# Tencent-RoboticsX/lifelike-agility-and-play

Measured on NVIDIA H100. Metric: env-steps/sec PMC mocap-tracking, higher is better.
Workload: dtype f32

## Files before the change

### __graft_entry__.py

```python
import os
import subprocess
import sys

ROOT = os.path.dirname(os.path.abspath(__file__))
if ROOT not in sys.path:
    sys.path.insert(0, ROOT)
CSRC = os.path.join(ROOT, "lifelike_agility_and_play_b200", "csrc")
CUDA_LIB = os.path.join(CSRC, "libllq_cuda.so")
NVCC_FLAGS = ["-gencode", "arch=compute_90a,code=sm_90a", "-lineinfo", "-O3", "-std=c++17", "-prec-div=false",
              "-prec-sqrt=false", "-ftz=true", "-Xcompiler", "-fPIC", "-shared"]


def _stale(target, sources):
    if not os.path.exists(target):
        return True
    t = os.path.getmtime(target)
    return any(os.path.getmtime(s) > t for s in sources)


def build(force=False):
    srcs = [os.path.join(CSRC, f) for f in ("llq_cuda.cu", "llq_kernels.cuh", "llq_step16.cuh", "llq_math.cuh")]
    srcs += [os.path.join(ROOT, "include", f) for f in ("llq.h", "llq_model_layout.h")]
    srcs.append(os.path.abspath(__file__))
    if force or _stale(CUDA_LIB, srcs):
        nvcc = os.environ.get("NVCC", "/usr/local/cuda/bin/nvcc")
        subprocess.check_call([nvcc] + NVCC_FLAGS + ["-o", CUDA_LIB, os.path.join(CSRC, "llq_cuda.cu")])
    pol_lib, pol_src = os.path.join(CSRC, "libllq_policy.so"), [os.path.join(CSRC, "llq_policy.cu"), os.path.join(CSRC, "llq_policy_hier.cu")]
    if force or _stale(pol_lib, pol_src + [os.path.join(CSRC, "llq_philox.cuh"), os.path.join(ROOT, "include", "llq_policy.h"),
                                           os.path.join(ROOT, "include", "llq.h"), os.path.abspath(__file__)]):
        nvcc = os.environ.get("NVCC", "/usr/local/cuda/bin/nvcc")
        flags = [f for f in NVCC_FLAGS if not f.startswith("-prec-") and not f.startswith("-ftz")]
        subprocess.check_call([nvcc] + flags + ["-o", pol_lib] + pol_src)
    from oracle import oracle as _oracle
    _oracle.build(force=force)
    import lifelike_agility_and_play_b200

# ... 53 lines not shown
```

### lifelike_agility_and_play_b200/csrc/llq_cuda.cu

```cuda
#include "../../include/llq.h"
#include "../../include/llq_model_layout.h"
#include "llq_kernels.cuh"
#include "llq_step16.cuh"

#include <cmath>
#include <cstdio>
#include <cstdlib>
#include <cstring>
#include <new>
#include <string>
#include <vector>

namespace {

thread_local std::string g_err;
int fail(int code, const std::string& msg) { g_err = msg; return code; }
#define CK(call)                                                                                         \
  do {                                                                                                   \
    cudaError_t e_ = (call);                                                                             \
    if (e_ != cudaSuccess) return fail(LLQ_ECUDA, std::string(#call) + ": " + cudaGetErrorString(e_));   \
  } while (0)

constexpr int kPadFrames = 128;

// ... 70 lines not shown
    h->h_scratch = nullptr; h->d_scratch = nullptr; h->h_scratch_bytes = 0;
    CK(cudaMallocHost(&h->h_scratch, bytes));
    CK(cudaMalloc(&h->d_scratch, bytes));
    h->h_scratch_bytes = h->d_scratch_bytes = bytes;
  }
  return LLQ_OK;
}

llq::MocapDev mocap_dev(llq_handle h) { return llq::MocapDev{h->d_frames, h->d_clip_off, h->n_clips, h->d_ob_table, h->d_ob_off}; }

template <int ENV>
void launch_reset_t(llq_handle h, const llq::EnvArrays& E, const llq::ResetParams& RP, float* obs2, long long ld, cudaStream_t s) {
  constexpr int BLOCK = llq::kResetBlock;
  int threads = 4 * h->cfg.n_envs;
  int grid = (threads + BLOCK - 1) / BLOCK;
  size_t smem = sizeof(double) * (size_t)(h->n_clips > 0 ? h->n_clips : 1);
  llq::pmc_reset_kernel<ENV><<<grid, BLOCK, smem, s>>>(E, mocap_dev(h), h->P, h->d_model, RP, obs2, ld);
}
template <int ENV>
int launch_step16(llq_handle h, const llq::EnvArrays& E, const float* a, float* obs2, long long ld, cudaStream_t s) {
  constexpr int EPB = LLQ16_BLOCK / 16;
  const int grid = (h->cfg.n_envs + EPB - 1) / EPB;
  const size_t smem = sizeof(float) * (EPB * llq::kEnvFloats + (LLQ16_BLOCK / 32) * llq::kATabWarp);
  const unsigned bit = 1u << (16 + ENV);
  if (!(h->smem_attr_set & bit)) {
    CK(cudaFuncSetAttribute(llq::llq_step16_kernel<ENV>, cudaFuncAttributeMaxDynamicSharedMemorySize, (int)smem));
    h->smem_attr_set |= bit;
  }
  llq::llq_step16_kernel<ENV><<<grid, LLQ16_BLOCK, smem, s>>>(E, mocap_dev(h), h->P, h->d_model, h->d_sph, a, obs2, ld, h->d_winner[h->parity],
                                                   (unsigned long long)h->cfg.seed, (long long)h->cfg.global_env_offset, h->record);
  return LLQ_OK;
// ... 630 lines not shown

int llq_sync(llq_handle h) {
  if (!h) return fail(LLQ_EINVAL, "null handle");
  int rc = set_device(h);
  if (rc) return rc;
  CK(cudaStreamSynchronize(h->stream));
  return LLQ_OK;
}

const char* llq_last_error(void) { return g_err.c_str(); }

}

#ifdef LLQ16_TIMING
extern "C" int llq_debug_timing(void* out, int n_warps) {
  return cudaMemcpyFromSymbol(out, llq::g_t16, (size_t)n_warps * 12 * sizeof(unsigned long long)) == cudaSuccess ? 0 : -1;
}
#endif
```

### lifelike_agility_and_play_b200/csrc/llq_kernels.cuh

```cuda
#pragma once
#include "../../include/llq.h"
#include "llq_math.cuh"
#include <cuda_pipeline.h>
#include <stdint.h>

namespace llq {

constexpr int kObsDim = 207, kObsDimEpmc = 916, kObsDimSepmc = 965, kPropDim = 33, kActDim = 12, kStateDim = 37, kAuxDim = 18;
template <int ENV> struct ObsW { static constexpr int value = (ENV == 1 || ENV == 3) ? kObsDimEpmc : (ENV == 2 ? kObsDimSepmc : kObsDim); };
constexpr int kMaxBoxes = 36, kMaxCand = 12;

constexpr int kNewObs = 120;
constexpr int kSQ = 0, kSQd = 12;
constexpr int kSPropBase = 24;
constexpr int kSAct = kPropDim;
constexpr int kSFuture = 45;
constexpr int kSRot = 45;
constexpr int kSPos = 54;
constexpr int kSTarget = 57;
constexpr int kSTargetSpd = 59;
constexpr int kSPosNorm = 60;
constexpr int kSCorrYaw = 61;
constexpr int kSMaskGrid = 62, kSMaskFront = 64, kSMaskLidar = 66;
constexpr int kSFlag = 57;
// ... 442 lines not shown
    snew[kSCorrYaw] = yaw;
    snew[kSMaskGrid] = __uint_as_float((unsigned)m2); snew[kSMaskGrid + 1] = __uint_as_float((unsigned)(m2 >> 32));
    snew[kSMaskFront] = __uint_as_float((unsigned)mf); snew[kSMaskFront + 1] = __uint_as_float((unsigned)(mf >> 32));
    snew[kSMaskLidar] = __uint_as_float((unsigned)m1); snew[kSMaskLidar + 1] = __uint_as_float((unsigned)(m1 >> 32));
  }
}
LLQ_DI unsigned long long staged_mask(const float* sn, int slot) {
  return ((unsigned long long)__float_as_uint(sn[slot + 1]) << 32) | __float_as_uint(sn[slot]);
}

struct ObsCtx {
  KinBase kb;
  float kq[3], kqd[3];
};

LLQ_DI ObsCtx build_obs_new(const MocapDev& mc, const StepParams& P, const ModelConst& M, int lane4, int clip, int frame_id,
                            double frac, double px, double py, double pz, Q4 qb, V3 lin, V3 ang, const float (&q)[3],
                            const float (&qd)[3], float* snew) {
  ObsCtx o;
  const MocapFrame* f0 = mc.frames + mc.clip_off[clip] + frame_id;
  o.kb = mocap_base(f0, f0 + 1, frac, P.frame_dt);
  float inv = (float)(1.0 / P.frame_dt), fr = (float)frac;
#pragma unroll
  for (int i = 0; i < 3; i++) {
    float c = f0->q[3 * lane4 + i], n = f0[1].q[3 * lane4 + i];
    o.kq[i] = fmaf(fr, n - c, c);
    o.kqd[i] = (n - c) * inv;
  }
  qb = qnormalize(qb);
  M3 Rb = qmat(qb);
  stage_joints(snew, lane4, q, qd);
  if (lane4 == 0) stage_prop_base(snew, Rb, tmul(Rb, ang), tmul(Rb, lin));
  {
    const double tf = lane4 == 0 ? 1. / 30. : (lane4 == 1 ? 1. / 15. : (lane4 == 2 ? 1. / 3. : 1.));
    double t = P.frame_dt * frac + tf;
    int fid = (int)floor(t / P.frame_dt);
    double ffrac = t / P.frame_dt - fid;
    const MocapFrame* g0 = f0 + fid;
    KinBase kf = mocap_base(g0, g0 + 1, ffrac, P.frame_dt);
    V3 dp = tmul(Rb, V3{(float)(kf.px - px), (float)(kf.py - py), (float)(kf.pz - pz)});
    V3 rv = q_rotvec(qnormalize(qmul(qconj(qb), qnormalize(kf.q))));
    float angle = norm3(rv);
    float sc = angle / (angle + 1e-8f);
    float* o18 = snew + kSFuture + 18 * lane4;
    o18[0] = dp.x; o18[1] = dp.y; o18[2] = dp.z;
    o18[3] = sc * rv.x; o18[4] = sc * rv.y; o18[5] = sc * rv.z;
    float ff = (float)ffrac;
#pragma unroll
    for (int j = 0; j < 12; j++) { float c = g0->q[j], n = g0[1].q[j]; o18[6 + j] = fmaf(ff, n - c, c); }
  }
  return o;
}

LLQ_DI M3 staged_rot(const float* sn) {
  const float* r = sn + kSRot;
  return M3{r[0], r[1], r[2], r[3], r[4], r[5], r[6], r[7], r[8]};
}
LLQ_DI float2 grid_point(const float* sn, int t) {
  const int a = t / 13, b = t - a * 13;
  const float gx = a == 24 ? 1.2f : -1.2f + (float)a * (2.4f / 24.0f), gy = b == 12 ? 0.6f : -0.6f + (float)b * (1.2f / 12.0f);
  const M3 R = staged_rot(sn);
  return make_float2(fmaf(R.a00, gx, fmaf(R.a01, gy, sn[kSPos])), fmaf(R.a10, gx, fmaf(R.a11, gy, sn[kSPos + 1])));
}
LLQ_DI V3 lidar_dir(float yaw, int t) {
// ... 134 lines not shown
LLQ_DI StartPose start_pose(const ModelConst& M, int k, double yaw_deg) {
  StartPose s;
  double sn, cs;
  sincos(0.5 * yaw_deg * (3.14159265358979323846 / 180.0), &sn, &cs);
  const float* I0 = M.init_state;
  s.qn = qmul(qnormalize(Q4{I0[3], I0[4], I0[5], I0[6]}), Q4{0.f, 0.f, (float)sn, (float)cs});
#pragma unroll
  for (int i = 0; i < 3; i++) { s.q[i] = I0[13 + 3 * k + i]; s.qd[i] = I0[25 + 3 * k + i]; }
  s.lin = V3{I0[7], I0[8], I0[9]}; s.ang = V3{I0[10], I0[11], I0[12]};
  const Q4 qI = Q4{M.base.qI[0], M.base.qI[1], M.base.qI[2], M.base.qI[3]};
  s.qp = qmul(qnormalize(s.qn), qconj(qI));
  return s;
}

constexpr int kResetBlock = 128;
template <int ENV>
__global__ void __launch_bounds__(kResetBlock) pmc_reset_kernel(EnvArrays E, MocapDev mc, StepParams P, const ModelConst* __restrict__ gmodel,
                                                                ResetParams RP, float* obs2, long long obs2_ld) {
  extern __shared__ double s_cdf[];
  __shared__ __align__(16) ModelConst M;
  __shared__ __align__(16) float s_new[kResetBlock / 4][kNewObs];
  prefetch_model(gmodel, &M, kResetBlock);
  __pipeline_commit();
  const int C = mc.n_clips;
  for (int c = threadIdx.x; c < C; c += kResetBlock) {
    double avg = RP.avg_old[c];
    if (RP.update_table) {
      int w = RP.winner_cur[c];
      if (w >= 0) avg = (double)E.done_reward[w] / RP.max_steps[c];
    }
    s_cdf[c] = avg;
  }
  __syncthreads();
  if (RP.update_table && blockIdx.x == 0)
    for (int c = threadIdx.x; c < C; c += kResetBlock) { RP.avg_new[c] = s_cdf[c]; RP.winner_next[c] = -1; }
  __syncthreads();
  for (int c = threadIdx.x; c < C; c += kResetBlock) s_cdf[c] = pow(1.0 - s_cdf[c], RP.factor);
  __syncthreads();
  __shared__ double s_tot;
  if (threadIdx.x == 0) {
    double tot = 0;
    for (int c = 0; c < C; c++) tot += s_cdf[c];
    s_tot = tot;
  }
  __syncthreads();
  for (int c = threadIdx.x; c < C; c += kResetBlock) {
    const double pc = s_cdf[c] / s_tot;
    s_cdf[c] = pc;
    if (blockIdx.x == 0) RP.prob[c] = pc;
  }
  __syncthreads();
  if (threadIdx.x == 0 && C > 0) {
    double acc = 0;
    for (int c = 0; c < C; c++) { acc += s_cdf[c]; s_cdf[c] = acc; }
    s_tot = s_cdf[C - 1];
  }
  __syncthreads();
  for (int c = threadIdx.x; c < C; c += kResetBlock) s_cdf[c] = s_cdf[c] / s_tot;
  __syncthreads();

  __pipeline_wait_prior(0);
  __syncthreads();
  const int N = P.n_envs;
  const int gtid = blockIdx.x * kResetBlock + threadIdx.x;
  const int env_raw = gtid >> 2;
  const int env = env_raw < N ? env_raw : N - 1;
  const bool valid = env_raw < N;
  const int k = threadIdx.x & 3;
  bool doit = valid;
  if (RP.mode == 3) doit = false;
  else if (RP.mode == 0) doit = doit && E.done[env] != 0;
  else if (RP.mask) doit = doit && (RP.mask[env] != 0 || (ENV == 2 && RP.mask[env ^ 1] != 0));
  const unsigned wm = __ballot_sync(FULL, doit);
  if (wm == 0) return;
  const LegConst& L = M.leg[k];

  if (ENV == 2) {
    const int robot = env & 1;
    const long long ep = E.episode[env & ~1];
    const long long gid = RP.gid0 + (env & ~1);
    double u0[4], u1[4], u2[4];
    stream_uniforms(RP.seed, gid, ep, 1, 0, u0);
    stream_uniforms(RP.seed, gid, ep, 1, 1, u1);
    stream_uniforms(RP.seed, gid, ep, 1, 2, u2);
    const float fix_spd = (float)(0.5 + 2.5 * u0[0]);
    const int wflag = (int)floor(2.0 * u0[1]);
    const double foot_mu = (double)P.fr_lo + u0[2] * ((double)P.fr_hi - (double)P.fr_lo);
    const double px = robot == 0 ? -2.0 + 4.0 * u0[3] : -2.0 + 4.0 * u1[1], py = robot == 0 ? -2.0 + 4.0 * u1[0] : -2.0 + 4.0 * u1[2];
    const double acc0 = E.aux[LLQ_AUX_YAW_ACCUM_DEG * N + (env & ~1)];
// ... 57 lines not shown
      write_reset(E, N, env, k, ep + 1);
      if (k == 0) {
        double* A = E.aux;
        A[LLQ_AUX_COUNTER * N + env] = 0; A[LLQ_AUX_CMD_FREQ * N + env] = cmd_freq; A[LLQ_AUX_TARGET_X * N + env] = tgx0;
        A[LLQ_AUX_TARGET_Y * N + env] = 0.0; A[LLQ_AUX_LAST_POS_DIFF_LEN * N + env] = fabs(tgx0); A[LLQ_AUX_TOTAL_SPD * N + env] = 0.0;
        A[LLQ_AUX_INIT_POS_DIFF_LEN * N + env] = fabs(tgx0);
        if (ENV == 3) E.nbox[env] = nb0;
        A[LLQ_AUX_MAX_SPD * N + env] = 0.0; A[LLQ_AUX_PUSH_COUNT * N + env] = P.push_start_count; A[LLQ_AUX_PUSH_F * N + env] = pf[0];
        A[(LLQ_AUX_PUSH_F + 1) * N + env] = pf[1]; A[(LLQ_AUX_PUSH_F + 2) * N + env] = pf[2];
        A[LLQ_AUX_FOOT_FRICTION * N + env] = foot_mu; A[LLQ_AUX_PUSH_DRAWS * N + env] = push_draws; A[LLQ_AUX_CMD_DRAWS * N + env] = 0;
        A[LLQ_AUX_YAW_ACCUM_DEG * N + env] = yaw_deg;
      }
    }
  } else {
    int clip; double t0;
    long long ep = E.episode[env];
    if (RP.mode == 2) {
      clip = RP.clip_in[env]; t0 = RP.time_in[env];
      if (!doit) { clip = 0; t0 = 0.0; }
    } else {
      long long gid = RP.gid0 + env;
      unsigned c4[4] = {(unsigned)gid, (unsigned)((unsigned long long)gid >> 32), (unsigned)ep, (unsigned)((unsigned long long)ep >> 32)};
      philox4x32_10(c4, (unsigned)RP.seed, (unsigned)(RP.seed >> 32));
      double u1 = ((double)c4[0] + 0.5) * (1.0 / 4294967296.0), u2 = ((double)c4[1] + 0.5) * (1.0 / 4294967296.0);
      clip = C - 1;
      for (int c = 0; c < C; c++) if (s_cdf[c] > u1) { clip = c; break; }
      int nf = mc.clip_off[clip + 1] - mc.clip_off[clip];
      t0 = u2 * (P.frame_dt * (double)(nf - P.margin - 1));
      ep += 1;
    }
    int frame_id = (int)floor(t0 / P.frame_dt);
    double frac = (t0 - frame_id * P.frame_dt) / P.frame_dt;
    {
      const int last = mc.clip_off[clip + 1] - mc.clip_off[clip] - P.margin + 2;
      if (frame_id > last) { frame_id = last; frac = 0.0; }
      if (frame_id < 0) { frame_id = 0; frac = 0.0; }
    }
    const MocapFrame* f0 = mc.frames + mc.clip_off[clip] + frame_id;
    KinBase kb = mocap_base(f0, f0 + 1, frac, P.frame_dt);
    float inv = (float)(1.0 / P.frame_dt), fr = (float)frac;
    float q[3], qd[3];
#pragma unroll
    for (int i = 0; i < 3; i++) {
      float c = f0->q[3 * k + i], n = f0[1].q[3 * k + i];
      q[i] = fmaf(fr, n - c, c);
      qd[i] = (n - c) * inv;
    }
    build_obs_new(mc, P, M, k, clip, frame_id, frac, kb.px, kb.py, kb.pz, kb.q, kb.lin, kb.ang, q, qd, s_new[threadIdx.x >> 2]);
    if (doit) {
      const Q4 qI = Q4{M.base.qI[0], M.base.qI[1], M.base.qI[2], M.base.qI[3]};
      const V3 fd = foot_world(L, qmul(qnormalize(kb.q), qconj(qI)), q, kb.px, kb.py, kb.pz);
      write_robot(E, N, env, k, q, qd, fd, kb.px, kb.py, kb.pz, kb.q, kb.lin, kb.ang, t0);
      write_reset(E, N, env, k, ep);
#pragma unroll
      for (int i = 0; i < 3; i++) { E.kin[(13 + 3 * k + i) * N + env] = q[i]; E.kin[(25 + 3 * k + i) * N + env] = qd[i]; }
      if (k == 0) {
        const float b[10] = {kb.q.x, kb.q.y, kb.q.z, kb.q.w, kb.lin.x, kb.lin.y, kb.lin.z, kb.ang.x, kb.ang.y, kb.ang.z};
        E.kin[env] = (float)kb.px; E.kin[N + env] = (float)kb.py; E.kin[2 * N + env] = (float)kb.pz;
#pragma unroll
        for (int i = 0; i < 10; i++) E.kin[(3 + i) * N + env] = b[i];
        E.clip[env] = clip;
        E.ob_id[env] = 0;
      }
    }
  }
  __syncwarp();
  unsigned rows = 0;
#pragma unroll
  for (int e = 0; e < 8; e++) if ((wm >> (4 * e)) & 1u) rows |= 1u << e;
  const int warp_env0 = (blockIdx.x * kResetBlock + (threadIdx.x & ~31)) >> 2;
  emit_obs_rows<ENV>(E.obs, obs2, obs2_ld, s_new[(threadIdx.x & ~31) >> 2], s_new[0], warp_env0, N, 1, rows, E.boxes);
}

}
```

### lifelike_agility_and_play_b200/csrc/llq_step16.cuh

```cuda
#pragma once
#include "llq_kernels.cuh"

namespace llq {

#ifndef LLQ16_BLOCK
#define LLQ16_BLOCK 256
#endif
#ifndef LLQ16_MINB
#define LLQ16_MINB 4
#endif
constexpr int kMaxSph = 32, kMaxCon = 8, kMaxLim = 8;
struct SphConst { float c[3]; float r; float mu_link; int leg; int depth; int foot; };
struct alignas(16) SphTable { int n; int rule; int pad[2]; SphConst s[kMaxSph]; };

constexpr int kLinkW = 8, kLinkTab = 12 * kLinkW;
constexpr int kLkC1 = 0, kLkS1 = 1, kLkCy = 2, kLkSy = 3, kLkP = 4;
constexpr int kLegW = 48, kLegTab = 4 * kLegW;
constexpr int kLgF = 0;
constexpr int kLgH = 18;
constexpr int kLgRhs = 27;
constexpr int kLgMass = 30, kLgMom = 31, kLgI = 34;
constexpr int kLgBias = 40;
constexpr int kLgW = 0;
constexpr int kLgL10 = 18, kLgL20 = 19, kLgL21 = 20;
// ... 5 lines not shown
constexpr int kCoDir = 5;
constexpr int kCoDist = 14, kCoMu = 15, kCoLam0 = 16;
constexpr int kCoLam = 17;
constexpr int kCoCone = 17, kCoLamT1 = 18, kCoLamT2 = 19;
constexpr int kLimW = 4, kLimTab = kMaxLim * kLimW;
constexpr int kLmLeg = 0, kLmJoint = 1, kLmDir = 2, kLmPen = 3;
constexpr int kRowW = 12, kRowTab = 32 * kRowW;
constexpr int kRwY = 0, kRwE = 6, kRwLeg = 9;
constexpr int kScrW = 20;
constexpr int kScBias = 0, kScMass = 6, kScMom = 7, kScI = 10;
constexpr int kResBase = 0, kResLeg = 6;
constexpr int kEnvTab = 56;
constexpr int kEvBias = 0;
constexpr int kEvVel = 0;
constexpr int kEvChol = 8;
constexpr int kEvTarget = 32, kEvAct = 44;
constexpr int kATabWarp = 32 * 32;
constexpr int kEnvFloats = 944;
static_assert(16 * kScrW <= kRowTab && kResLeg + 4 * 3 <= kRowTab, "the row table's other uses fit in it");
constexpr int kLinkOff = 0, kLegOff = kLinkOff + kLinkTab, kConOff = kLegOff + kLegTab, kLimOff = kConOff + kConTab;
constexpr int kRowOff = kLimOff + kLimTab, kEnvOff = kRowOff + kRowTab;
static_assert(kEnvOff + kEnvTab <= kEnvFloats && kEnvFloats % 32 == 16, "per-env table layout");
struct LegFrames {
  float c1, s1, c2, s2, c23, s23;
  V3 p1, p2, p3;
  LLQ_DI V3 on_thigh(V3 c) const { return p2 + rot<0>(rot<1>(c, c2, s2), c1, s1); }
  LLQ_DI V3 on_shank(V3 c) const { return p3 + rot<0>(rot<1>(c, c23, s23), c1, s1); }
};
LLQ_DI LegFrames leg_frames(const float* link, int k) {
  const float* lk = link + 3 * k * kLinkW;
// ... 72 lines not shown
    const double len = sqrt(v0 * v0 + v1 * v1 + v2 * v2);
    db = len - r;
    nn = V3{(float)(v0 / len), (float)(v1 / len), (float)(v2 / len)};
  } else {
    double best = h0 - p0; nn = V3{1.f, 0.f, 0.f};
    if (h0 + p0 < best) { best = h0 + p0; nn = V3{-1.f, 0.f, 0.f}; }
    if (h1 - p1 < best) { best = h1 - p1; nn = V3{0.f, 1.f, 0.f}; }
    if (h1 + p1 < best) { best = h1 + p1; nn = V3{0.f, -1.f, 0.f}; }
    if (h2 - p2 < best) { best = h2 - p2; nn = V3{0.f, 0.f, 1.f}; }
    if (h2 + p2 < best) { best = h2 + p2; nn = V3{0.f, 0.f, -1.f}; }
    db = -best - r;
  }
}

#ifdef LLQ16_TIMING
__device__ unsigned long long g_t16[16384 * 12];
#define T16_DECL long long t16_[12] = {0, 0, 0, 0, 0, 0, 0, 0, 0, 0, 0, 0}, t16_c = clock64(), t16_s = t16_c
#define T16_MARK(slot) { const long long t16_n = clock64(); t16_[slot] += t16_n - t16_c; t16_c = t16_n; }
#define T16_ADD(slot, v) t16_[slot] += (v)
#define T16_IN(slot) { const long long t16_n = clock64(); in.t16[slot] += t16_n - *in.t16c; *in.t16c = t16_n; }
#else
#define T16_DECL
#define T16_MARK(slot)
#define T16_ADD(slot, v)
#define T16_IN(slot)
#endif
struct RowsIn {
#ifdef LLQ16_TIMING
  long long* t16; long long* t16c;
#endif
  float* tb;
  float* acol;
  int nc, nl;
  int rr;
  int lane0;
  int lane;
  int split;
  int Cmax, Lmax;
  float* res;
  float dt, slop, erp, jerp, max_imp;
// ... 213 lines not shown
        if (s == at_fric) { r.lam = nown; rc = nown + r.rhs; }
        r.b = fmaf(ap[32], na - la, fmaf(ap[64], nb - lb, r.b));
      }
    }
  }
#undef LLQ16_ROW_UPDATE
#undef LLQ16_CLAMP_LIMIT
#undef LLQ16_CLAMP_NORMAL
  T16_IN(10);
  if (is_normal) in.tb[kConOff + (in.rr / 3) * kConW + kCoLam] = r.lam;
  __syncwarp();
  impulse_sums(in, r);
  T16_IN(3);
}

struct TailState {
  double px, py, pz, time, frame_frac;
  int frame_id, ob_id, flags, push_count, push_draws;
  float pf[3], qp[4], vw[3], ww[3], q[12], qd[12];
};
static_assert(sizeof(TailState) <= sizeof(float) * kRowTab, "the hand-over record lives in the row table");
LLQ_DI bool fallen(const M3& R) {
  const float left_z = R.a02 * R.a10 - R.a12 * R.a00;
  return left_z > 0.70710678118654752f || left_z < -0.70710678118654752f || R.a22 < 0.5f;
}
template <int ENV>
LLQ_DI void step_tail(const EnvArrays& E, const MocapDev& mc, const StepParams& P, const ModelConst& M, float* s_new, const float* s_hist,
                      const TailState& T, const float* act_src, float* obs2, long long obs2_ld, int* winner, unsigned long long seed, long long gid0,
                      int record, int el, int k, int env, bool valid) {
  const int N = P.n_envs;
  double px = T.px, py = T.py, pz = T.pz, time = T.time, frame_frac = T.frame_frac;
  int frame_id = T.frame_id, ob_id = T.ob_id, push_count = T.push_count, push_draws = T.push_draws;
  bool bad = (T.flags & 1) != 0, ob_hit = (T.flags & 2) != 0;
  const bool touch_own = (T.flags & 4) != 0, tag = (T.flags & 8) != 0;
  const float pf[3] = {T.pf[0], T.pf[1], T.pf[2]};
  const Q4 qp = Q4{T.qp[0], T.qp[1], T.qp[2], T.qp[3]};
  const V3 vw = V3{T.vw[0], T.vw[1], T.vw[2]}, ww = V3{T.ww[0], T.ww[1], T.ww[2]};
  float q[3], qd[3];
#pragma unroll
  for (int t = 0; t < 3; t++) { q[t] = T.q[3 * k + t]; qd[t] = T.qd[3 * k + t]; }
  const int clip = ENV == 0 ? E.clip[env] : 0;
  const long long epi = ENV != 0 ? E.episode[ENV == 2 ? env & ~1 : env] - 1 : 0;
  const int robot = env & 1;
  const long long pair_gid = gid0 + (env & ~1);
  bool done = false;
  float rew_out = 0.f;
  const bool wr = valid;
  const LegConst& L = M.leg[k];
  const Q4 qI = Q4{M.base.qI[0], M.base.qI[1], M.base.qI[2], M.base.qI[3]};
  const Q4 qb = qmul(qp, qI);
  PairState PS = {0, 0, 1, 0, 0.0, 0.0};
  if (ENV == 0) {
    float* snew = s_new + el * kNewObs;
    ObsCtx oc = build_obs_new(mc, P, M, k, clip, frame_id, frame_frac, px, py, pz, qb, vw, ww, q, qd, snew);
#pragma unroll
    for (int t = 0; t < 3; t++) snew[kSAct + 3 * k + t] = act_src[3 * k + t];
    float djp = 0.f, djv = 0.f;
#pragma unroll
    for (int t = 0; t < 3; t++) { float a = q[t] - oc.kq[t], b = qd[t] - oc.kqd[t]; djp = fmaf(a, a, djp); djv = fmaf(b, b, djv); }
    V3 f;
    const V3 fd = foot_world(L, qp, q, px, py, pz, &f);
    const V3 g = mul(qmat(qmul(qnormalize(oc.kb.q), qconj(qI))), foot_in_base(L, oc.kq[0], oc.kq[1], oc.kq[2]));
    const V3 fk = V3{(float)(oc.kb.px - px) + g.x - f.x, (float)(oc.kb.py - py) + g.y - f.y, (float)(oc.kb.pz - pz) + g.z - f.z};
    float dee = dot(fk, fk);
    djp = gsum4(djp); djv = gsum4(djv); dee = gsum4(dee);
    float dpx = (float)(px - oc.kb.px), dpy = (float)(py - oc.kb.py), dpz = (float)(pz - oc.kb.pz);
    float dp = dpx * dpx + dpy * dpy + dpz * dpz;
    V3 dvl3 = vw - oc.kb.lin, dva3 = ww - oc.kb.ang;
    Q4 q1 = qnormalize(qb), q2 = qnormalize(oc.kb.q);
    float angle = norm3(q_rotvec(qnormalize(qmul(q2, qconj(q1)))));
    float rew = P.w_jp * expf(-1.0f * djp) + P.w_jv * expf(-0.1f * djv) + P.w_ee * expf(-40.0f * dee) +
                P.w_pose * expf(-20.0f * dp - 10.0f * angle * angle) + P.w_vel * expf(-2.0f * dot(dvl3, dvl3) - 0.2f * dot(dva3, dva3));
    const bool fall = fallen(qmat(q1));
    int nf = mc.clip_off[clip + 1] - mc.clip_off[clip];
    bool ended = frame_id >= nf - P.margin - 1;
    bool diff = fabsf(angle) > 1.0f || dp > 1.0f;
    if (bad || !isfinite(rew)) { rew = 0.f; bad = true; }
    if (P.has_ob) {
      int oh = ob_hit ? 1 : 0;
      oh |= __shfl_xor_sync(FULL, oh, 1);
      oh |= __shfl_xor_sync(FULL, oh, 2);
      ob_hit = oh != 0;
      const int o0 = mc.ob_off[clip], n_ob = mc.ob_off[clip + 1] - o0;
      while (ob_id < n_ob - 1 && time > mc.ob_table[(size_t)(o0 + ob_id) * 4] + 0.5) ob_id++;
    }
    done = fall || ended || diff || ob_hit || bad;
    rew_out = rew;
    if (wr) {
      write_robot(E, N, env, k, q, qd, fd, px, py, pz, qb, vw, ww, time);
// ... 12 lines not shown
        }
      }
    }
  } else if (ENV == 2) {
    const double* A = E.aux;
    int counter = (int)A[LLQ_AUX_COUNTER * N + env];
    PS.with_flag = (int)A[LLQ_AUX_WITH_FLAG * N + env]; PS.flag_x = A[LLQ_AUX_FLAG_X * N + env]; PS.flag_y = A[LLQ_AUX_FLAG_Y * N + env];
    const float fix_spd = (float)A[LLQ_AUX_CONTROL_SPD * N + env];
    double total_spd = A[LLQ_AUX_TOTAL_SPD * N + env], max_spd = A[LLQ_AUX_MAX_SPD * N + env];
    PS.flag_draws = (int)A[LLQ_AUX_FLAG_DRAWS * N + env];
    float* snew = s_new + el * kNewObs;
    const float* spart = s_new + (el ^ 1) * kNewObs;
    sepmc_pair_tail(M, L, k, robot, snew, spart, px, py, pz, qp, qb, vw, ww, q, touch_own, fix_spd, seed, pair_gid, epi, PS);
    stage_joints(snew, k, q, qd);
#pragma unroll
    for (int t = 0; t < 3; t++) snew[kSAct + 3 * k + t] = act_src[3 * k + t];
    const float spd = sqrtf(vw.x * vw.x + vw.y * vw.y);
    total_spd += (double)spd;
    if ((double)spd > max_spd) max_spd = (double)spd;
    counter += 1;
    int fall = fallen(qmat(qnormalize(qb))) ? 1 : 0;
    const int fall_other = __shfl_xor_sync(FULL, fall, 4);
    if (robot == 1) fall = fall_other;
    const int bad_other = __shfl_xor_sync(FULL, bad ? 1 : 0, 4);
    bad = bad || bad_other != 0;
    done = fall != 0 || counter >= P.max_steps || tag || bad;
    const int wf0 = robot == 0 ? PS.with_flag : 1 - PS.with_flag;
    float rew = (float)PS.sw * ((wf0 != 0) == (robot == 0) ? 1.f : -1.f);
    if (done && tag) rew += (wf0 != 0) == (robot == 0) ? 1.f : -1.f;
    if (bad) rew = 0.f;
    rew_out = rew;
// ... 29 lines not shown
          double sn, cs;
          sincos(target_angle, &sn, &cs);
          tgx = sx0 + cs * 100.0; tgy = sy0 + sn * 100.0;
          last_len = sqrt((sx0 - tgx) * (sx0 - tgx) + (sy0 - tgy) * (sy0 - tgy));
        }
        target_spd = (float)((double)P.ts_lo + uu[1] * ((double)P.ts_hi - (double)P.ts_lo));
      }
      if (ENV == 3) target_angle = atan2(tgy - sy0, tgx - sx0);
    }
    __syncwarp();
    float* snew = s_new + el * kNewObs;
    const Q4 q1 = qnormalize(qb);
    const M3 Rq = qmat(q1);
    stage_joints(snew, k, q, qd);
#pragma unroll
    for (int t = 0; t < 3; t++) snew[kSAct + 3 * k + t] = act_src[3 * k + t];
    counter += 1;
    const double dx = tgx - px, dy = tgy - py;
    const double plen = sqrt(dx * dx + dy * dy);
    if (k == 0) {
      stage_pose(snew, Rq, tmul(Rq, ww), tmul(Rq, vw), V3{(float)px, (float)py, (float)pz});
      stage_target(snew, Rq, px, py, pz, tgx, tgy, target_spd);
    }
    const bool fall = fallen(Rq);
    const bool reach = plen < 0.5, timeup = counter >= P.max_steps;
    const float ux = (float)(dx / plen), uy = (float)(dy / plen);
    const float spd = fabsf(vw.x * ux + vw.y * uy);
    total_spd += (double)spd;
    if ((double)spd > max_spd) max_spd = (double)spd;
    const float yaw = atan2f(Rq.a10, Rq.a00);
    float sy_, cy_;
// ... 16 lines not shown
      if (k == 0) {
        write_step(E, env, rew, done);
        double* Aw = E.aux;
        Aw[LLQ_AUX_COUNTER * N + env] = counter; Aw[LLQ_AUX_CMD_FREQ * N + env] = cmd_freq; Aw[LLQ_AUX_TARGET_X * N + env] = tgx;
        Aw[LLQ_AUX_TARGET_Y * N + env] = tgy; Aw[LLQ_AUX_TARGET_SPD * N + env] = target_spd;
        Aw[LLQ_AUX_TARGET_ANGLE * N + env] = target_angle; Aw[LLQ_AUX_LAST_POS_DIFF_LEN * N + env] = last_len;
        Aw[LLQ_AUX_TOTAL_SPD * N + env] = total_spd; Aw[LLQ_AUX_MAX_SPD * N + env] = max_spd;
        Aw[LLQ_AUX_PUSH_COUNT * N + env] = push_count; Aw[LLQ_AUX_PUSH_F * N + env] = pf[0]; Aw[(LLQ_AUX_PUSH_F + 1) * N + env] = pf[1]; Aw[(LLQ_AUX_PUSH_F + 2) * N + env] = pf[2];
        Aw[LLQ_AUX_PUSH_DRAWS * N + env] = push_draws; Aw[LLQ_AUX_CMD_DRAWS * N + env] = cmd_draws;
      }
    }
  }
  if (record && obs2 && wr) {
    float* row = obs2 + (size_t)env * obs2_ld + ObsW<ENV>::value - (record == 2 ? (long long)N * obs2_ld : 0ll);
#pragma unroll
    for (int t = 0; t < 3; t++) row[3 * k + t] = act_src[3 * k + t];
    if (k == 0) { row[12] = rew_out; row[13] = done ? 1.f : 0.f; }
  }
  {
    const unsigned dm = __ballot_sync(FULL, valid && k == 0 && done);
    if ((threadIdx.x & 31) == 0 && dm) atomicAdd(&E.counters[1], (unsigned long long)__popc(dm));
  }
}

template <int ENV>
__global__ void __launch_bounds__(LLQ16_BLOCK, LLQ16_MINB * 128 / LLQ16_BLOCK) llq_step16_kernel(EnvArrays E, MocapDev mc, StepParams P, const ModelConst* __restrict__ gmodel,
                                                            const SphTable* __restrict__ gsph, const float* __restrict__ actions,
                                                            float* obs2, long long obs2_ld, int* __restrict__ winner,
                                                            unsigned long long seed, long long gid0, int record) {
  constexpr int BLOCK = LLQ16_BLOCK, EPB = BLOCK / 16;
  constexpr int EPT = (EPB + 7) / 8 * 8;
// ... 48 lines not shown
  for (int t = 0; t < 3; t++) {
    q[t] = st[(10 + 3 * k + t) * N + env];
    qd[t] = st[(22 + 3 * k + t) * N + env];
  }
  if (i < 3) {
    const float a = actions[(size_t)env * kActDim + 3 * k + i];
    envtab[kEvAct + 3 * k + i] = a;
    envtab[kEvTarget + 3 * k + i] = clampf((i == 0 ? q[0] : (i == 1 ? q[1] : q[2])) + a, -3.0f, 3.0f);
  }
  const int nsph = ST.n, rule = ST.rule;
  float warm[2];
  warm[0] = l16 < nsph ? E.warm[(size_t)l16 * N + env] : 0.f;
  warm[1] = 16 + l16 < nsph ? E.warm[(size_t)(16 + l16) * N + env] : 0.f;
  double time = E.time[env];
  const int clip = ENV == 0 ? E.clip[env] : 0;
  int frame_id = 0; double frame_frac = 0.0;
  int ob_id = 0; bool ob_hit = false;
  if (ENV == 0 && P.has_ob) ob_id = E.ob_id[env];
  int push_count = 0, push_draws = 0;
  float pf[3] = {0.f, 0.f, 0.f}, mu_env = P.mu;
  long long epi = 0;
  PairState PS = {0, 0, 1, 0, 0.0, 0.0};
  bool touch_own = false, tag = false;
  const int robot = env & 1;
  const long long pair_gid = gid0 + (env & ~1);
  if (ENV != 0) {
    const double* A = E.aux;
    push_count = (int)A[LLQ_AUX_PUSH_COUNT * N + env];
    pf[0] = (float)A[LLQ_AUX_PUSH_F * N + env]; pf[1] = (float)A[(LLQ_AUX_PUSH_F + 1) * N + env]; pf[2] = (float)A[(LLQ_AUX_PUSH_F + 2) * N + env];
    mu_env = P.mu_ground * (float)A[LLQ_AUX_FOOT_FRICTION * N + env]; push_draws = (int)A[LLQ_AUX_PUSH_DRAWS * N + env];
// ... 551 lines not shown
      }
      px += (double)vw.x * P.sim_dt; py += (double)vw.y * P.sim_dt; pz += (double)vw.z * P.sim_dt;
      float fa = norm3(ww);
      float sc;
      sc = 0.5f * dt - dt * dt * dt * 0.020833333333f * fa * fa;
      float sh, chh;
      llq_sincosf(0.5f * fa * dt, &sh, &chh);
      if (!(fa < 0.001f)) sc = sh / fa;
      Q4 dq = Q4{sc * ww.x, sc * ww.y, sc * ww.z, chh};
      qp = qnormalize(qmul(dq, qp));
    }
    bad = bad || !(fabsf(qd[0]) <= P.vmax) || !(fabsf(ww.x) <= P.vmax) || !(fabsf(vw.x) <= P.vmax) || !isfinite(q[0] + q[1] + q[2]);
    if (ENV == 0 && sub == P.substeps - 1) {
      frame_id = (int)floor(time / P.frame_dt);
      frame_frac = (time - frame_id * P.frame_dt) / P.frame_dt;
      const int last = mc.clip_off[clip + 1] - mc.clip_off[clip] - P.margin + 2;
      if (frame_id > last) { frame_id = last; frame_frac = 0.0; }
      if (frame_id < 0) { frame_id = 0; frame_frac = 0.0; }
    }
    time += P.sim_dt;
  }
  __syncwarp();

  {
    int bi = bad ? 1 : 0;
    bi |= __shfl_xor_sync(FULL, bi, 1); bi |= __shfl_xor_sync(FULL, bi, 2); bi |= __shfl_xor_sync(FULL, bi, 4); bi |= __shfl_xor_sync(FULL, bi, 8);
    bad = bi != 0;
  }
  if (valid) {
    if (l16 < nsph) E.warm[(size_t)l16 * N + env] = warm[0];
    if (16 + l16 < nsph) E.warm[(size_t)(16 + l16) * N + env] = warm[1];
// ... 23 lines not shown
    if ((threadIdx.x & 31) == 0) {
      if (cr) atomicAdd(&E.counters[2], (unsigned long long)cr);
      if (lr) atomicAdd(&E.counters[3], (unsigned long long)lr);
      if (ov) atomicAdd(&E.counters[5], (unsigned long long)ov);
    }
  }
  __pipeline_wait_prior(0);
  __syncthreads();
  if (tid < 4 * EPT) {
    const int tel = tid >> 2, tk = tid & 3;
    const bool tval = tel < EPB && blockIdx.x * EPB + tel < N;
    const int tsrc = tel < EPB ? tel : EPB - 1;
    const int tenv_raw = blockIdx.x * EPB + tsrc;
    const float* tbase = s_env_dyn + tsrc * kEnvFloats;
    step_tail<ENV>(E, mc, P, M, s_new[0], s_hist[0], *reinterpret_cast<const TailState*>(tbase + kRowOff),
                   tbase + (kEnvOff + kEvAct), obs2, obs2_ld, winner, seed, gid0, record, tel, tk, tenv_raw < N ? tenv_raw : N - 1, tval);
  }
  __syncthreads();
  emit_obs_rows<ENV, 2>(E.obs, obs2, obs2_ld, s_new[(tid >> 5) << 1], s_hist[(tid >> 5) << 1], warp_env0, N, 0, 0x3u, E.boxes);
#ifdef LLQ16_TIMING
  T16_MARK(4);
  t16_[7] = clock64() - t16_s;
  if ((tid & 31) == 0) {
    const int gw = blockIdx.x * (BLOCK / 32) + (tid >> 5);
    if (gw < 16384) for (int t = 0; t < 12; t++) g_t16[gw * 12 + t] = (unsigned long long)t16_[t];
  }
#endif
}

}
```

Before: 16.77 million.

## Streamline reset CDF build, binary-search clip sampling, and prefetch mocap frames

The reset kernel now fuses the clip-weight computation passes, exits early for blocks with no env to reset, vectorizes the serial sum and prefix scan with double2, and replaces the linear CDF scan with a binary search. Clip offsets are cached in shared memory. The step kernel stashes clip offsets in the per-env shared table and issues L2 prefetches for the mocap frames the tail will read, so that latency overlaps with the substep physics. Future-frame loads in build_obs_new are hoisted earlier, and timing-probe scaffolding is added behind macros, at the cost of extra prefetch instructions and some code complexity.

New measurement: 17.26 million (median of 6 runs). 2.9% higher.

```diff
diff --git a/__graft_entry__.py b/__graft_entry__.py
--- a/__graft_entry__.py
+++ b/__graft_entry__.py
@@ -19,7 +19,7 @@
 
 
 def build(force=False):
-    srcs = [os.path.join(CSRC, f) for f in ("llq_cuda.cu", "llq_kernels.cuh", "llq_step16.cuh", "llq_math.cuh")]
+    srcs = [os.path.join(CSRC, f) for f in ("llq_cuda.cu", "llq_kernels.cuh", "llq_step16.cuh", "llq_math.cuh", "llq_cdf.h")]
     srcs += [os.path.join(ROOT, "include", f) for f in ("llq.h", "llq_model_layout.h")]
     srcs.append(os.path.abspath(__file__))
     if force or _stale(CUDA_LIB, srcs):
diff --git a/lifelike_agility_and_play_b200/csrc/llq_cdf.h b/lifelike_agility_and_play_b200/csrc/llq_cdf.h
--- /dev/null
+++ b/lifelike_agility_and_play_b200/csrc/llq_cdf.h
@@ -0,0 +1,18 @@
+#pragma once
+#if defined(__CUDACC__)
+#define LLQ_HD_INLINE __host__ __device__ __forceinline__
+#else
+#define LLQ_HD_INLINE inline
+#endif
+
+namespace llq {
+LLQ_HD_INLINE int cdf_search(const double* cdf, int C, double u) {
+  int lo = 0, hi = C - 1;
+  while (lo < hi) {
+    const int mid = (lo + hi) >> 1;
+    if (cdf[mid] > u) hi = mid;
+    else lo = mid + 1;
+  }
+  return hi;
+}
+}
diff --git a/lifelike_agility_and_play_b200/csrc/llq_cuda.cu b/lifelike_agility_and_play_b200/csrc/llq_cuda.cu
--- a/lifelike_agility_and_play_b200/csrc/llq_cuda.cu
+++ b/lifelike_agility_and_play_b200/csrc/llq_cuda.cu
@@ -108,7 +108,7 @@
   constexpr int BLOCK = llq::kResetBlock;
   int threads = 4 * h->cfg.n_envs;
   int grid = (threads + BLOCK - 1) / BLOCK;
-  size_t smem = sizeof(double) * (size_t)(h->n_clips > 0 ? h->n_clips : 1);
+  const size_t smem = sizeof(double) * (size_t)(h->n_clips > 0 ? h->n_clips : 1) + sizeof(int) * (size_t)(h->n_clips + 1);
   llq::pmc_reset_kernel<ENV><<<grid, BLOCK, smem, s>>>(E, mocap_dev(h), h->P, h->d_model, RP, obs2, ld);
 }
 template <int ENV>
@@ -769,6 +769,11 @@
 
 #ifdef LLQ16_TIMING
 extern "C" int llq_debug_timing(void* out, int n_warps) {
-  return cudaMemcpyFromSymbol(out, llq::g_t16, (size_t)n_warps * 12 * sizeof(unsigned long long)) == cudaSuccess ? 0 : -1;
+  return cudaMemcpyFromSymbol(out, llq::g_t16, (size_t)n_warps * 13 * sizeof(unsigned long long)) == cudaSuccess ? 0 : -1;
 }
 #endif
+#ifdef LLQ_RESET_TIMING
+extern "C" int llq_debug_reset_timing(void* out, int n_warps) {
+  return cudaMemcpyFromSymbol(out, llq::g_tr, (size_t)n_warps * 6 * sizeof(unsigned long long)) == cudaSuccess ? 0 : -1;
+}
+#endif
diff --git a/lifelike_agility_and_play_b200/csrc/llq_kernels.cuh b/lifelike_agility_and_play_b200/csrc/llq_kernels.cuh
--- a/lifelike_agility_and_play_b200/csrc/llq_kernels.cuh
+++ b/lifelike_agility_and_play_b200/csrc/llq_kernels.cuh
@@ -1,6 +1,7 @@
 #pragma once
 #include "../../include/llq.h"
 #include "llq_math.cuh"
+#include "llq_cdf.h"
 #include <cuda_pipeline.h>
 #include <stdint.h>
 
@@ -480,12 +481,31 @@
   float kq[3], kqd[3];
 };
 
-LLQ_DI ObsCtx build_obs_new(const MocapDev& mc, const StepParams& P, const ModelConst& M, int lane4, int clip, int frame_id,
-                            double frac, double px, double py, double pz, Q4 qb, V3 lin, V3 ang, const float (&q)[3],
-                            const float (&qd)[3], float* snew) {
+LLQ_DI int future_frame(const StepParams& P, double frac, int lane4, double& ffrac) {
+  const double tf = lane4 == 0 ? 1. / 30. : (lane4 == 1 ? 1. / 15. : (lane4 == 2 ? 1. / 3. : 1.));
+  const double t = P.frame_dt * frac + tf;
+  const int fid = (int)floor(t / P.frame_dt);
+  ffrac = t / P.frame_dt - fid;
+  return fid;
+}
+LLQ_DI void prefetch_frame_pair(const MocapFrame* f) {
+  const char* p = reinterpret_cast<const char*>(f);
+  asm volatile("prefetch.global.L2 [%0];" :: "l"(p));
+  asm volatile("prefetch.global.L2 [%0];" :: "l"(p + 128));
+  asm volatile("prefetch.global.L2 [%0];" :: "l"(p + 2 * sizeof(MocapFrame) - 1));
+}
+
+LLQ_DI ObsCtx build_obs_new(const MocapFrame* f0, const StepParams& P, const ModelConst& M, int lane4, double frac, double px,
+                            double py, double pz, Q4 qb, V3 lin, V3 ang, const float (&q)[3], const float (&qd)[3], float* snew) {
   ObsCtx o;
-  const MocapFrame* f0 = mc.frames + mc.clip_off[clip] + frame_id;
+  double ffrac;
+  const MocapFrame* g0 = f0 + future_frame(P, frac, lane4, ffrac);
   o.kb = mocap_base(f0, f0 + 1, frac, P.frame_dt);
+  const KinBase kf = mocap_base(g0, g0 + 1, ffrac, P.frame_dt);
+  float gq[12];
+  const float ff = (float)ffrac;
+#pragma unroll
+  for (int j = 0; j < 12; j++) { float c = g0->q[j], n = g0[1].q[j]; gq[j] = fmaf(ff, n - c, c); }
   float inv = (float)(1.0 / P.frame_dt), fr = (float)frac;
 #pragma unroll
   for (int i = 0; i < 3; i++) {
@@ -498,12 +518,6 @@
   stage_joints(snew, lane4, q, qd);
   if (lane4 == 0) stage_prop_base(snew, Rb, tmul(Rb, ang), tmul(Rb, lin));
   {
-    const double tf = lane4 == 0 ? 1. / 30. : (lane4 == 1 ? 1. / 15. : (lane4 == 2 ? 1. / 3. : 1.));
-    double t = P.frame_dt * frac + tf;
-    int fid = (int)floor(t / P.frame_dt);
-    double ffrac = t / P.frame_dt - fid;
-    const MocapFrame* g0 = f0 + fid;
-    KinBase kf = mocap_base(g0, g0 + 1, ffrac, P.frame_dt);
     V3 dp = tmul(Rb, V3{(float)(kf.px - px), (float)(kf.py - py), (float)(kf.pz - pz)});
     V3 rv = q_rotvec(qnormalize(qmul(qconj(qb), qnormalize(kf.q))));
     float angle = norm3(rv);
@@ -511,9 +525,8 @@
     float* o18 = snew + kSFuture + 18 * lane4;
     o18[0] = dp.x; o18[1] = dp.y; o18[2] = dp.z;
     o18[3] = sc * rv.x; o18[4] = sc * rv.y; o18[5] = sc * rv.z;
-    float ff = (float)ffrac;
-#pragma unroll
-    for (int j = 0; j < 12; j++) { float c = g0->q[j], n = g0[1].q[j]; o18[6 + j] = fmaf(ff, n - c, c); }
+#pragma unroll
+    for (int j = 0; j < 12; j++) o18[6 + j] = gq[j];
   }
   return o;
 }
@@ -678,53 +691,30 @@
 }
 
 constexpr int kResetBlock = 128;
+#ifdef LLQ_RESET_TIMING
+constexpr int kResetTimingWarps = 8192;
+__device__ unsigned long long g_tr[kResetTimingWarps * 6];
+#define TR_DECL long long tr_[6] = {0, 0, 0, 0, 0, 0}, tr_c = clock64(), tr_s = tr_c
+#define TR_MARK(slot) { const long long tr_n = clock64(); tr_[slot] += tr_n - tr_c; tr_c = tr_n; }
+#define TR_STORE() { tr_[5] = clock64() - tr_s; const int gw_ = (blockIdx.x * kResetBlock + threadIdx.x) >> 5; \
+    if ((threadIdx.x & 31) == 0 && gw_ < kResetTimingWarps) for (int t_ = 0; t_ < 6; t_++) g_tr[gw_ * 6 + t_] = (unsigned long long)tr_[t_]; }
+#else
+#define TR_DECL
+#define TR_MARK(slot)
+#define TR_STORE()
+#endif
 template <int ENV>
 __global__ void __launch_bounds__(kResetBlock) pmc_reset_kernel(EnvArrays E, MocapDev mc, StepParams P, const ModelConst* __restrict__ gmodel,
                                                                 ResetParams RP, float* obs2, long long obs2_ld) {
-  extern __shared__ double s_cdf[];
+  extern __shared__ __align__(16) double s_cdf[];
   __shared__ __align__(16) ModelConst M;
   __shared__ __align__(16) float s_new[kResetBlock / 4][kNewObs];
+  __shared__ double s_tot;
+  TR_DECL;
   prefetch_model(gmodel, &M, kResetBlock);
   __pipeline_commit();
   const int C = mc.n_clips;
-  for (int c = threadIdx.x; c < C; c += kResetBlock) {
-    double avg = RP.avg_old[c];
-    if (RP.update_table) {
-      int w = RP.winner_cur[c];
-      if (w >= 0) avg = (double)E.done_reward[w] / RP.max_steps[c];
-    }
-    s_cdf[c] = avg;
-  }
-  __syncthreads();
-  if (RP.update_table && blockIdx.x == 0)
-    for (int c = threadIdx.x; c < C; c += kResetBlock) { RP.avg_new[c] = s_cdf[c]; RP.winner_next[c] = -1; }
-  __syncthreads();
-  for (int c = threadIdx.x; c < C; c += kResetBlock) s_cdf[c] = pow(1.0 - s_cdf[c], RP.factor);
-  __syncthreads();
-  __shared__ double s_tot;
-  if (threadIdx.x == 0) {
-    double tot = 0;
-    for (int c = 0; c < C; c++) tot += s_cdf[c];
-    s_tot = tot;
-  }
-  __syncthreads();
-  for (int c = threadIdx.x; c < C; c += kResetBlock) {
-    const double pc = s_cdf[c] / s_tot;
-    s_cdf[c] = pc;
-    if (blockIdx.x == 0) RP.prob[c] = pc;
-  }
-  __syncthreads();
-  if (threadIdx.x == 0 && C > 0) {
-    double acc = 0;
-    for (int c = 0; c < C; c++) { acc += s_cdf[c]; s_cdf[c] = acc; }
-    s_tot = s_cdf[C - 1];
-  }
-  __syncthreads();
-  for (int c = threadIdx.x; c < C; c += kResetBlock) s_cdf[c] = s_cdf[c] / s_tot;
-  __syncthreads();
-
-  __pipeline_wait_prior(0);
-  __syncthreads();
+  int* const s_off = reinterpret_cast<int*>(s_cdf + C);
   const int N = P.n_envs;
   const int gtid = blockIdx.x * kResetBlock + threadIdx.x;
   const int env_raw = gtid >> 2;
@@ -735,8 +725,75 @@
   if (RP.mode == 3) doit = false;
   else if (RP.mode == 0) doit = doit && E.done[env] != 0;
   else if (RP.mask) doit = doit && (RP.mask[env] != 0 || (ENV == 2 && RP.mask[env ^ 1] != 0));
+  long long ep0 = 0; int clip_in = 0; double time_in = 0.0;
+  double u_clip = 0.0, u_time = 0.0;
+  if (ENV == 0) {
+    ep0 = E.episode[env];
+    if (RP.mode == 2) {
+      clip_in = RP.clip_in[env]; time_in = RP.time_in[env];
+    } else {
+      const long long gid = RP.gid0 + env;
+      unsigned c4[4] = {(unsigned)gid, (unsigned)((unsigned long long)gid >> 32), (unsigned)ep0, (unsigned)((unsigned long long)ep0 >> 32)};
+      philox4x32_10(c4, (unsigned)RP.seed, (unsigned)(RP.seed >> 32));
+      u_clip = ((double)c4[0] + 0.5) * (1.0 / 4294967296.0); u_time = ((double)c4[1] + 0.5) * (1.0 / 4294967296.0);
+    }
+    for (int c = threadIdx.x; c <= C; c += kResetBlock) s_off[c] = mc.clip_off[c];
+  }
+  const bool table = blockIdx.x == 0 || RP.mode < 2;
+  if (table) {
+    for (int c = threadIdx.x; c < C; c += kResetBlock) {
+      double avg = RP.avg_old[c];
+      if (RP.update_table) {
+        const int w = RP.winner_cur[c];
+        if (w >= 0) avg = (double)E.done_reward[w] / RP.max_steps[c];
+        if (blockIdx.x == 0) { RP.avg_new[c] = avg; RP.winner_next[c] = -1; }
+      }
+      s_cdf[c] = pow(1.0 - avg, RP.factor);
+    }
+  }
+  const bool any = __syncthreads_or(doit) != 0;
+  TR_MARK(1);
+  if (!any && blockIdx.x != 0) { TR_STORE(); return; }
+  if (table) {
+    const double2* s2 = reinterpret_cast<const double2*>(s_cdf);
+    if (threadIdx.x == 0) {
+      double tot = 0;
+      int c = 0;
+#pragma unroll 4
+      for (; c + 1 < C; c += 2) { const double2 v = s2[c >> 1]; tot += v.x; tot += v.y; }
+      if (c < C) tot += s_cdf[c];
+      s_tot = tot;
+    }
+    __syncthreads();
+    for (int c = threadIdx.x; c < C; c += kResetBlock) {
+      const double pc = s_cdf[c] / s_tot;
+      s_cdf[c] = pc;
+      if (blockIdx.x == 0) RP.prob[c] = pc;
+    }
+    __syncthreads();
+    if (threadIdx.x == 0 && C > 0) {
+      double2* d2 = reinterpret_cast<double2*>(s_cdf);
+      double acc = 0;
+      int c = 0;
+#pragma unroll 4
+      for (; c + 1 < C; c += 2) {
+        const double2 v = s2[c >> 1];
+        acc += v.x;
+        const double a0 = acc;
+        acc += v.y;
+        d2[c >> 1] = make_double2(a0, acc);
+      }
+      if (c < C) { acc += s_cdf[c]; s_cdf[c] = acc; }
+      s_tot = acc;
+    }
+    __syncthreads();
+    for (int c = threadIdx.x; c < C; c += kResetBlock) s_cdf[c] = s_cdf[c] / s_tot;
+  }
+  __pipeline_wait_prior(0);
+  __syncthreads();
+  TR_MARK(0);
   const unsigned wm = __ballot_sync(FULL, doit);
-  if (wm == 0) return;
+  if (wm == 0) { TR_STORE(); return; }
   const LegConst& L = M.leg[k];
 
   if (ENV == 2) {
@@ -824,29 +881,29 @@
     }
   } else {
     int clip; double t0;
-    long long ep = E.episode[env];
+    long long ep = ep0;
     if (RP.mode == 2) {
-      clip = RP.clip_in[env]; t0 = RP.time_in[env];
+      clip = clip_in; t0 = time_in;
       if (!doit) { clip = 0; t0 = 0.0; }
     } else {
-      long long gid = RP.gid0 + env;
-      unsigned c4[4] = {(unsigned)gid, (unsigned)((unsigned long long)gid >> 32), (unsigned)ep, (unsigned)((unsigned long long)ep >> 32)};
-      philox4x32_10(c4, (unsigned)RP.seed, (unsigned)(RP.seed >> 32));
-      double u1 = ((double)c4[0] + 0.5) * (1.0 / 4294967296.0), u2 = ((double)c4[1] + 0.5) * (1.0 / 4294967296.0);
-      clip = C - 1;
-      for (int c = 0; c < C; c++) if (s_cdf[c] > u1) { clip = c; break; }
-      int nf = mc.clip_off[clip + 1] - mc.clip_off[clip];
-      t0 = u2 * (P.frame_dt * (double)(nf - P.margin - 1));
+      clip = cdf_search(s_cdf, C, u_clip);
+      TR_MARK(2);
+      int nf = s_off[clip + 1] - s_off[clip];
+      t0 = u_time * (P.frame_dt * (double)(nf - P.margin - 1));
       ep += 1;
     }
     int frame_id = (int)floor(t0 / P.frame_dt);
     double frac = (t0 - frame_id * P.frame_dt) / P.frame_dt;
     {
-      const int last = mc.clip_off[clip + 1] - mc.clip_off[clip] - P.margin + 2;
+      const int last = s_off[clip + 1] - s_off[clip] - P.margin + 2;
       if (frame_id > last) { frame_id = last; frac = 0.0; }
       if (frame_id < 0) { frame_id = 0; frac = 0.0; }
     }
-    const MocapFrame* f0 = mc.frames + mc.clip_off[clip] + frame_id;
+    const MocapFrame* f0 = mc.frames + s_off[clip] + frame_id;
+    {
+      double ffrac;
+      prefetch_frame_pair(f0 + future_frame(P, frac, k, ffrac));
+    }
     KinBase kb = mocap_base(f0, f0 + 1, frac, P.frame_dt);
     float inv = (float)(1.0 / P.frame_dt), fr = (float)frac;
     float q[3], qd[3];
@@ -856,7 +913,7 @@
       q[i] = fmaf(fr, n - c, c);
       qd[i] = (n - c) * inv;
     }
-    build_obs_new(mc, P, M, k, clip, frame_id, frac, kb.px, kb.py, kb.pz, kb.q, kb.lin, kb.ang, q, qd, s_new[threadIdx.x >> 2]);
+    build_obs_new(f0, P, M, k, frac, kb.px, kb.py, kb.pz, kb.q, kb.lin, kb.ang, q, qd, s_new[threadIdx.x >> 2]);
     if (doit) {
       const Q4 qI = Q4{M.base.qI[0], M.base.qI[1], M.base.qI[2], M.base.qI[3]};
       const V3 fd = foot_world(L, qmul(qnormalize(kb.q), qconj(qI)), q, kb.px, kb.py, kb.pz);
@@ -875,11 +932,14 @@
     }
   }
   __syncwarp();
+  TR_MARK(3);
   unsigned rows = 0;
 #pragma unroll
   for (int e = 0; e < 8; e++) if ((wm >> (4 * e)) & 1u) rows |= 1u << e;
   const int warp_env0 = (blockIdx.x * kResetBlock + (threadIdx.x & ~31)) >> 2;
   emit_obs_rows<ENV>(E.obs, obs2, obs2_ld, s_new[(threadIdx.x & ~31) >> 2], s_new[0], warp_env0, N, 1, rows, E.boxes);
-}
-
-}
+  TR_MARK(4);
+  TR_STORE();
+}
+
+}
diff --git a/lifelike_agility_and_play_b200/csrc/llq_step16.cuh b/lifelike_agility_and_play_b200/csrc/llq_step16.cuh
--- a/lifelike_agility_and_play_b200/csrc/llq_step16.cuh
+++ b/lifelike_agility_and_play_b200/csrc/llq_step16.cuh
@@ -43,6 +43,7 @@
 constexpr int kEvBias = 0;
 constexpr int kEvVel = 0;
 constexpr int kEvChol = 8;
+constexpr int kEvClipOff = 29, kEvClipEnd = 30;
 constexpr int kEvTarget = 32, kEvAct = 44;
 constexpr int kATabWarp = 32 * 32;
 constexpr int kEnvFloats = 944;
@@ -145,16 +146,22 @@
 }
 
 #ifdef LLQ16_TIMING
-__device__ unsigned long long g_t16[16384 * 12];
-#define T16_DECL long long t16_[12] = {0, 0, 0, 0, 0, 0, 0, 0, 0, 0, 0, 0}, t16_c = clock64(), t16_s = t16_c
+__device__ unsigned long long g_t16[16384 * 13];
+#define T16_DECL long long t16_[13] = {0, 0, 0, 0, 0, 0, 0, 0, 0, 0, 0, 0, 0}, t16_c = clock64(), t16_s = t16_c
 #define T16_MARK(slot) { const long long t16_n = clock64(); t16_[slot] += t16_n - t16_c; t16_c = t16_n; }
 #define T16_ADD(slot, v) t16_[slot] += (v)
 #define T16_IN(slot) { const long long t16_n = clock64(); in.t16[slot] += t16_n - *in.t16c; *in.t16c = t16_n; }
+#define T16_TAIL_PARAMS , long long* t16, long long* t16c
+#define T16_TAIL_ARGS , t16_, &t16_c
+#define T16_TAIL(slot) { const long long t16_n = clock64(); t16[slot] += t16_n - *t16c; *t16c = t16_n; }
 #else
 #define T16_DECL
 #define T16_MARK(slot)
 #define T16_ADD(slot, v)
 #define T16_IN(slot)
+#define T16_TAIL_PARAMS
+#define T16_TAIL_ARGS
+#define T16_TAIL(slot)
 #endif
 struct RowsIn {
 #ifdef LLQ16_TIMING
@@ -398,6 +405,26 @@
   T16_IN(3);
 }
 
+LLQ_DI void prefetch_tail_frames(const MocapFrame* clip0, const StepParams& P, int nf, double time, int l16) {
+  for (int s = 0; s < P.substeps - 1; s++) time += P.sim_dt;
+  int frame_id = (int)floor(time / P.frame_dt);
+  double frac = (time - frame_id * P.frame_dt) / P.frame_dt;
+  const int last = nf - P.margin + 2;
+  if (frame_id > last) { frame_id = last; frac = 0.0; }
+  if (frame_id < 0) { frame_id = 0; frac = 0.0; }
+  if (l16 < 5) {
+    int f = frame_id;
+    if (l16 < 4) {
+      const double tf = l16 == 0 ? 1. / 30. : (l16 == 1 ? 1. / 15. : (l16 == 2 ? 1. / 3. : 1.));
+      f += (int)floor((P.frame_dt * frac + tf) / P.frame_dt);
+    }
+    const char* p = reinterpret_cast<const char*>(clip0 + f);
+    asm volatile("prefetch.global.L2 [%0];" :: "l"(p));
+    asm volatile("prefetch.global.L2 [%0];" :: "l"(p + 128));
+    asm volatile("prefetch.global.L2 [%0];" :: "l"(p + 2 * sizeof(MocapFrame) - 1));
+  }
+}
+
 struct TailState {
   double px, py, pz, time, frame_frac;
   int frame_id, ob_id, flags, push_count, push_draws;
@@ -410,8 +437,8 @@
 }
 template <int ENV>
 LLQ_DI void step_tail(const EnvArrays& E, const MocapDev& mc, const StepParams& P, const ModelConst& M, float* s_new, const float* s_hist,
-                      const TailState& T, const float* act_src, float* obs2, long long obs2_ld, int* winner, unsigned long long seed, long long gid0,
-                      int record, int el, int k, int env, bool valid) {
+                      const TailState& T, const float* ev, float* obs2, long long obs2_ld, int* winner, unsigned long long seed, long long gid0,
+                      int record, int el, int k, int env, bool valid T16_TAIL_PARAMS) {
   const int N = P.n_envs;
   double px = T.px, py = T.py, pz = T.pz, time = T.time, frame_frac = T.frame_frac;
   int frame_id = T.frame_id, ob_id = T.ob_id, push_count = T.push_count, push_draws = T.push_draws;
@@ -436,9 +463,11 @@
   PairState PS = {0, 0, 1, 0, 0.0, 0.0};
   if (ENV == 0) {
     float* snew = s_new + el * kNewObs;
-    ObsCtx oc = build_obs_new(mc, P, M, k, clip, frame_id, frame_frac, px, py, pz, qb, vw, ww, q, qd, snew);
-#pragma unroll
-    for (int t = 0; t < 3; t++) snew[kSAct + 3 * k + t] = act_src[3 * k + t];
+    const int off0 = __float_as_int(ev[kEvClipOff]);
+    ObsCtx oc = build_obs_new(mc.frames + off0 + frame_id, P, M, k, frame_frac, px, py, pz, qb, vw, ww, q, qd, snew);
+    T16_TAIL(12);
+#pragma unroll
+    for (int t = 0; t < 3; t++) snew[kSAct + 3 * k + t] = ev[kEvAct + 3 * k + t];
     float djp = 0.f, djv = 0.f;
 #pragma unroll
     for (int t = 0; t < 3; t++) { float a = q[t] - oc.kq[t], b = qd[t] - oc.kqd[t]; djp = fmaf(a, a, djp); djv = fmaf(b, b, djv); }
@@ -456,7 +485,7 @@
     float rew = P.w_jp * expf(-1.0f * djp) + P.w_jv * expf(-0.1f * djv) + P.w_ee * expf(-40.0f * dee) +
                 P.w_pose * expf(-20.0f * dp - 10.0f * angle * angle) + P.w_vel * expf(-2.0f * dot(dvl3, dvl3) - 0.2f * dot(dva3, dva3));
     const bool fall = fallen(qmat(q1));
-    int nf = mc.clip_off[clip + 1] - mc.clip_off[clip];
+    int nf = __float_as_int(ev[kEvClipEnd]) - off0;
     bool ended = frame_id >= nf - P.margin - 1;
     bool diff = fabsf(angle) > 1.0f || dp > 1.0f;
     if (bad || !isfinite(rew)) { rew = 0.f; bad = true; }
@@ -499,7 +528,7 @@
     sepmc_pair_tail(M, L, k, robot, snew, spart, px, py, pz, qp, qb, vw, ww, q, touch_own, fix_spd, seed, pair_gid, epi, PS);
     stage_joints(snew, k, q, qd);
 #pragma unroll
-    for (int t = 0; t < 3; t++) snew[kSAct + 3 * k + t] = act_src[3 * k + t];
+    for (int t = 0; t < 3; t++) snew[kSAct + 3 * k + t] = ev[kEvAct + 3 * k + t];
     const float spd = sqrtf(vw.x * vw.x + vw.y * vw.y);
     total_spd += (double)spd;
     if ((double)spd > max_spd) max_spd = (double)spd;
@@ -559,7 +588,7 @@
     const M3 Rq = qmat(q1);
     stage_joints(snew, k, q, qd);
 #pragma unroll
-    for (int t = 0; t < 3; t++) snew[kSAct + 3 * k + t] = act_src[3 * k + t];
+    for (int t = 0; t < 3; t++) snew[kSAct + 3 * k + t] = ev[kEvAct + 3 * k + t];
     counter += 1;
     const double dx = tgx - px, dy = tgy - py;
     const double plen = sqrt(dx * dx + dy * dy);
@@ -606,7 +635,7 @@
   if (record && obs2 && wr) {
     float* row = obs2 + (size_t)env * obs2_ld + ObsW<ENV>::value - (record == 2 ? (long long)N * obs2_ld : 0ll);
 #pragma unroll
-    for (int t = 0; t < 3; t++) row[3 * k + t] = act_src[3 * k + t];
+    for (int t = 0; t < 3; t++) row[3 * k + t] = ev[kEvAct + 3 * k + t];
     if (k == 0) { row[12] = rew_out; row[13] = done ? 1.f : 0.f; }
   }
   {
@@ -685,6 +714,11 @@
   warm[1] = 16 + l16 < nsph ? E.warm[(size_t)(16 + l16) * N + env] : 0.f;
   double time = E.time[env];
   const int clip = ENV == 0 ? E.clip[env] : 0;
+  if (ENV == 0) {
+    const int off0 = mc.clip_off[clip], off1 = mc.clip_off[clip + 1];
+    if (l16 == 0) { envtab[kEvClipOff] = __int_as_float(off0); envtab[kEvClipEnd] = __int_as_float(off1); }
+    prefetch_tail_frames(mc.frames + off0, P, off1 - off0, time, l16);
+  }
   int frame_id = 0; double frame_frac = 0.0;
   int ob_id = 0; bool ob_hit = false;
   if (ENV == 0 && P.has_ob) ob_id = E.ob_id[env];
@@ -1266,7 +1300,7 @@
     if (ENV == 0 && sub == P.substeps - 1) {
       frame_id = (int)floor(time / P.frame_dt);
       frame_frac = (time - frame_id * P.frame_dt) / P.frame_dt;
-      const int last = mc.clip_off[clip + 1] - mc.clip_off[clip] - P.margin + 2;
+      const int last = __float_as_int(envtab[kEvClipEnd]) - __float_as_int(envtab[kEvClipOff]) - P.margin + 2;
       if (frame_id > last) { frame_id = last; frame_frac = 0.0; }
       if (frame_id < 0) { frame_id = 0; frame_frac = 0.0; }
     }
@@ -1320,7 +1354,8 @@
     const int tenv_raw = blockIdx.x * EPB + tsrc;
     const float* tbase = s_env_dyn + tsrc * kEnvFloats;
     step_tail<ENV>(E, mc, P, M, s_new[0], s_hist[0], *reinterpret_cast<const TailState*>(tbase + kRowOff),
-                   tbase + (kEnvOff + kEvAct), obs2, obs2_ld, winner, seed, gid0, record, tel, tk, tenv_raw < N ? tenv_raw : N - 1, tval);
+                   tbase + kEnvOff, obs2, obs2_ld, winner, seed, gid0, record, tel, tk, tenv_raw < N ? tenv_raw : N - 1, tval
+                   T16_TAIL_ARGS);
   }
   __syncthreads();
   emit_obs_rows<ENV, 2>(E.obs, obs2, obs2_ld, s_new[(tid >> 5) << 1], s_hist[(tid >> 5) << 1], warp_env0, N, 0, 0x3u, E.boxes);
@@ -1329,7 +1364,7 @@
   t16_[7] = clock64() - t16_s;
   if ((tid & 31) == 0) {
     const int gw = blockIdx.x * (BLOCK / 32) + (tid >> 5);
-    if (gw < 16384) for (int t = 0; t < 12; t++) g_t16[gw * 12 + t] = (unsigned long long)t16_[t];
+    if (gw < 16384) for (int t = 0; t < 13; t++) g_t16[gw * 13 + t] = (unsigned long long)t16_[t];
   }
 #endif
 }
```
